# lucasjinreal/yolov7_d2

Hardware: AMD Instinct MI355X
Metric: images/sec training, YOLOX-s 640x640 bs=16/GPU (higher is better)
Workload: dtype bf16; 1 GPU; YOLOX-s CSPDarknet+PAFPN 640x640 bs=16/GPU: fwd + SimOTA loss + bwd + grad all-reduce + SGD(momentum) step, uint8 image batch + labels resident in HBM; global_batch=16, parallelism=dp1, hipgraph=True

## Files before the change

yolov7_d2_amd/csrc/conv1x1_stream.h:

```cpp
#pragma once
#include "common.h"
#include "conv_bn.h"

#define C1_MAX_SLICES 16
#define C1_MAX_BN 2
struct C1Slice {
  const u32x4* w;
  __bf16* y;
  double* stats;
  int wld, ldy, sld, nslots;
  int bnj, c0;
  const float* bias;
  const __bf16* aux;
  int ldaux, pad2_;
};
struct C1K {
  const __bf16* x;
  int ldx, ntiles, nco, nb;
  int xcd_order, dbg;
  C1Slice s[C1_MAX_SLICES];
  CBnFwd bn[C1_MAX_BN];
  const BnXf* xf;
  int xfw, pad_;
  int relu, epi;
  int npix, ragged;
};
struct C1Launch {
  int K, WM, PT, NBUF, MODE, grid, lds, XF;
  C1K k;
};

#define C1_VMCNT(n) asm volatile("s_waitcnt vmcnt(%0)" ::"n"(n) : "memory")

static __device__ uint4 g_c1_zero_page[4];
static __device__ __attribute__((aligned(256))) unsigned g_c1_bar[MI_BN_BAR_WORDS];

__device__ __forceinline__ void c1_glds16(const void* sbase, unsigned voff, unsigned lds_off) {
  asm volatile("s_mov_b32 m0, %2\n\ts_nop 4\n\tglobal_load_lds_dwordx4 %0, %1" ::"v"(voff), "s"(sbase),
               "s"(lds_off)
               : "memory");
}

template <int K, int WM, int WN, int PT, int NBUF, int MODE, int XF = 0>
__global__ __launch_bounds__(WM* WN * 64) void c1s_kernel(const C1K p) {
  static_assert(!XF || MODE == 1, "the input transform comes with the forward (statistics) mode");
  constexpr int NW = WM * WN, TPIX = WN * PT * 32, KC8 = K / 8, KS = K / 16, R = K * 2;
  constexpr int XB = TPIX * R;
  constexpr int D = XB / (1024 * NW);
  static_assert(D >= 1 && XB % (1024 * NW) == 0, "tile / DMA split");
  constexpr int RPI = KC8 >= 64 ? 1 : 64 / KC8;
  constexpr int RBSH = K >= 128 ? 0 : (K == 64 ? 1 : 2);
  constexpr int SWM = KC8 - 1 < 15 ? KC8 - 1 : 15;
  constexpr int S = 2 * PT;
  constexpr bool AUXM = MODE == 2 || MODE == 5 || MODE == 6;
  constexpr bool RAGGED_OK = (MODE == 0 || MODE == 2 || MODE >= 4) && !XF;
  constexpr bool BIASM = MODE == 4 || MODE == 5;
  constexpr int L = MODE == 6 ? 4 * PT : (AUXM ? 2 * PT : 0);
  constexpr int W0 = (NBUF - 2) * D + L;
  constexpr int W1 = NBUF > 2 ? (NBUF - 2) * D + (S + L) + L : (S + L);
  constexpr int W2 = NBUF > 3 ? (NBUF - 2) * D + 2 * (S + L) + L : (NBUF - 2) * D + (NBUF - 1) * (S + L);
  constexpr int W3 = (NBUF - 2) * D + (NBUF - 1) * (S + L);
  static_assert(W3 < 64 && W2 < 64, "vmcnt field");
  constexpr int X1 = NBUF > 2 ? (NBUF - 3) * D + (2 * D + S) : S;
  constexpr int X2 = NBUF > 3 ? (NBUF - 4) * D + 2 * (2 * D + S) : (NBUF - 1) * S + (NBUF - 2) * 2 * D;
  constexpr int X3 = (NBUF - 1) * S + (NBUF - 2) * 2 * D;
  static_assert(!XF || (X3 < 64 && X2 < 64 && X1 < 64), "vmcnt field");

  extern __shared__ __attribute__((aligned(16))) char smem[];
  const unsigned lds0 = (unsigned)(uintptr_t)(__attribute__((address_space(3))) char*)smem;
  const int tid = threadIdx.x, lane = tid & 63;
  const int wave = __builtin_amdgcn_readfirstlane(tid >> 6);
  const int wm = wave / WN, wn = wave % WN;
  const int l31 = lane & 31, h = lane >> 5;
  const int nb = p.nb;
  const int cot = p.xcd_order ? (int)blockIdx.x / nb : (int)blockIdx.x % p.nco;
  const int b = p.xcd_order ? (int)blockIdx.x % nb : (int)blockIdx.x / p.nco;
  const int nt = (p.ntiles - b + nb - 1) / nb;
  const C1Slice sl = p.s[cot * WM + wm];
  unsigned gen0 = 0;
  if constexpr (MODE == 3) {
    const int nblk = (int)gridDim.x;
    if (tid == 0)
      gen0 = __hip_atomic_load(bn_bar_gen(g_c1_bar, (int)blockIdx.x % (nblk < BN_BAR_G ? nblk : BN_BAR_G)), __ATOMIC_RELAXED, __HIP_MEMORY_SCOPE_AGENT);
  }
  constexpr bool STATS = MODE == 1 || MODE == 3;

  bf16x8 a[KS];
#pragma unroll
  for (int ks = 0; ks < KS; ++ks) a[ks] = __builtin_bit_cast(bf16x8, sl.w[(size_t)(ks * 2 + h) * sl.wld + l31]);

  const int ldxb = p.ldx * 2;
  unsigned doff[D];
#pragma unroll
  for (int d = 0; d < D; ++d) {
    const int q = wave * D + d;
    const int row = q * RPI + (KC8 >= 64 ? 0 : lane / KC8);
    const int c = KC8 >= 64 ? lane : lane % KC8;
    doff[d] = (unsigned)(row * ldxb + ((c ^ ((row >> RBSH) & SWM)) << 4));
  }
  const size_t xtile = (size_t)TPIX * (size_t)ldxb;
  auto issue_x = [&](int i, int buf) {
    const bool live = i < nt;
    const char* xt = live ? (const char*)p.x + (size_t)(b + i * nb) * xtile : (const char*)g_c1_zero_page;
    if (RAGGED_OK && live && p.ragged && b + i * nb == p.ntiles - 1) {
      const int lim = p.npix - (p.ntiles - 1) * TPIX;
#pragma unroll
      for (int d = 0; d < D; ++d) {
        const int q = wave * D + d;
        const int row = q * RPI + (KC8 >= 64 ? 0 : lane / KC8);
        const int c = KC8 >= 64 ? lane : lane % KC8;
        c1_glds16(xt, row < lim ? doff[d] : (unsigned)(c << 4), lds0 + buf * XB + (wave * D + d) * 1024);
      }
      return;
    }
#pragma unroll
    for (int d = 0; d < D; ++d) c1_glds16(xt, live ? doff[d] : 0u, lds0 + buf * XB + (wave * D + d) * 1024);
  };

  unsigned brow[PT], bsw[PT];
#pragma unroll
  for (int j = 0; j < PT; ++j) {
    const int r = (wn * PT + j) * 32 + l31;
    brow[j] = (unsigned)(r * R);
    bsw[j] = (unsigned)((h ^ ((r >> RBSH) & SWM)) << 4);
  }
  const int ldyb = sl.ldy * 2;
  unsigned yoff[PT];
#pragma unroll
  for (int j = 0; j < PT; ++j) yoff[j] = (unsigned)(((wn * PT + j) * 32 + l31) * ldyb + h * 16);
  const size_t ytile = (size_t)TPIX * (size_t)ldyb;
  const int ldab5 = (MODE == 5 || MODE == 6) ? sl.ldaux * 2 : 0;
  unsigned aoff5[PT];
#pragma unroll
  for (int j = 0; j < PT; ++j) aoff5[j] = (unsigned)(((wn * PT + j) * 32 + l31) * ldab5 + h * 16);
  const size_t atile5 = (size_t)TPIX * (size_t)ldab5;
  float bs[BIASM ? 16 : 1];
  if constexpr (BIASM) {
#pragma unroll
    for (int q = 0; q < 4; ++q)
#pragma unroll
      for (int e = 0; e < 4; ++e) bs[4 * q + e] = sl.bias ? sl.bias[8 * q + 4 * h + e] : 0.f;
  }
  const bool relu4 = BIASM && p.relu != 0;

  float s1[16], s2[16];
  if constexpr (STATS) {
#pragma unroll
    for (int r = 0; r < 16; ++r) s1[r] = s2[r] = 0.f;
  }

#pragma unroll
  for (int i = 0; i < NBUF - 1; ++i) issue_x(i, i);

  float* const s_sc = (float*)(smem + NBUF * XB);
  float* const s_sh = s_sc + K;
  int xf_act = 0, xf_ldab = 0;
  char* xf_a = nullptr;
  if constexpr (XF) {
    bnx_tables(p.xf, s_sc, s_sh, NW * 64, blockIdx.x == 0);
    xf_act = p.xf->bn.act;
    xf_ldab = p.xf->bn.lda * 2;
    xf_a = (p.xfw && cot == 0) ? (char*)p.xf->bn.a : nullptr;
    __syncthreads();
  }

  int buf = 0, nbuf = NBUF - 1;
  for (int i = 0; i < nt; ++i) {
    char* const yt = (char*)sl.y + (size_t)(b + i * nb) * ytile;
    int lim = TPIX;
    if constexpr (RAGGED_OK) {
      if (p.ragged && b + i * nb == p.ntiles - 1) lim = p.npix - (p.ntiles - 1) * TPIX;
    }
    u32x4 old[2 * PT];
    u32x4 aux6[MODE == 6 ? 2 * PT : 1];
    if constexpr (MODE == 2 || MODE == 6) {
#pragma unroll
      for (int j = 0; j < PT; ++j) {
        const unsigned yo = ((wn * PT + j) * 32 + l31) < lim ? yoff[j] : (unsigned)(h * 16);
        asm volatile("s_nop 4\n\tglobal_load_dwordx4 %0, %1, %2" : "=v"(old[j * 2]) : "v"(yo), "s"(yt) : "memory");
        asm volatile("global_load_dwordx4 %0, %1, %2 offset:32" : "=v"(old[j * 2 + 1]) : "v"(yo), "s"(yt) : "memory");
      }
    }
    if constexpr (MODE == 5) {
      const char* const at5 = (const char*)sl.aux + (size_t)(b + i * nb) * atile5;
#pragma unroll
      for (int j = 0; j < PT; ++j) {
        const unsigned ao = ((wn * PT + j) * 32 + l31) < lim ? aoff5[j] : (unsigned)(h * 16);
        asm volatile("s_nop 4\n\tglobal_load_dwordx4 %0, %1, %2" : "=v"(old[j * 2]) : "v"(ao), "s"(at5) : "memory");
        asm volatile("global_load_dwordx4 %0, %1, %2 offset:32" : "=v"(old[j * 2 + 1]) : "v"(ao), "s"(at5) : "memory");
      }
    }
    if constexpr (MODE == 6) {
      const char* const at5 = (const char*)sl.aux + (size_t)(b + i * nb) * atile5;
#pragma unroll
      for (int j = 0; j < PT; ++j) {
        const unsigned ao = ((wn * PT + j) * 32 + l31) < lim ? aoff5[j] : (unsigned)(h * 16);
        asm volatile("s_nop 4\n\tglobal_load_dwordx4 %0, %1, %2" : "=v"(aux6[j * 2]) : "v"(ao), "s"(at5) : "memory");
        asm volatile("global_load_dwordx4 %0, %1, %2 offset:32" : "=v"(aux6[j * 2 + 1]) : "v"(ao), "s"(at5) : "memory");
      }
    }
    if (XF && xf_a) {
      if (i == 0) C1_VMCNT(W0);
      else if (i == 1) C1_VMCNT(X1);
      else if (i == 2) C1_VMCNT(X2);
      else C1_VMCNT(X3);
    } else {
      if (i == 0) C1_VMCNT(W0);
      else if (i == 1) C1_VMCNT(W1);
      else if (i == 2) C1_VMCNT(W2);
      else C1_VMCNT(W3);
    }
    if constexpr (XF) {
      char* const Xw = smem + buf * XB;
      char* const at = xf_a + (size_t)(b + i * nb) * ((size_t)TPIX * (size_t)xf_ldab);
#pragma unroll 2
      for (int d = 0; d < D; ++d) {
        const int q = wave * D + d;
        const int row = q * RPI + (KC8 >= 64 ? 0 : lane / KC8);
        const int c = KC8 >= 64 ? lane : lane % KC8;
        const int cg = c ^ ((row >> RBSH) & SWM);
        const u32x4 o = bnx_apply_lds(Xw + q * 1024 + lane * 16, s_sc, s_sh, cg, xf_act, true);
        if (xf_a) *(u32x4*)(at + (unsigned)(row * xf_ldab + cg * 16)) = o;
      }
      asm volatile("s_waitcnt lgkmcnt(0)" ::: "memory");
    }
    __builtin_amdgcn_s_barrier();
    issue_x(i + NBUF - 1, nbuf);

    f32x16 acc[PT];
#pragma unroll
    for (int j = 0; j < PT; ++j)
#pragma unroll
      for (int r = 0; r < 16; ++r) acc[j][r] = 0.f;
    const char* Xs = smem + buf * XB;
#pragma unroll
    for (int ks = 0; ks < KS; ++ks) {
      bf16x8 bf[PT];
#pragma unroll
      for (int j = 0; j < PT; ++j) bf[j] = __builtin_bit_cast(bf16x8, *(const u32x4*)(Xs + brow[j] + ((unsigned)(ks * 32) ^ bsw[j])));
#pragma unroll
      for (int j = 0; j < PT; ++j) acc[j] = __builtin_amdgcn_mfma_f32_32x32x16_bf16(a[ks], bf[j], acc[j], 0, 0, 0);
    }

    if constexpr (AUXM) {
      if constexpr (MODE == 6) {
        if constexpr (PT == 1)
          asm volatile("s_waitcnt vmcnt(%4)" : "+v"(old[0]), "+v"(old[1]), "+v"(aux6[0]), "+v"(aux6[1]) : "n"(D) : "memory");
        else
          asm volatile("s_waitcnt vmcnt(%8)"
                       : "+v"(old[0]), "+v"(old[1]), "+v"(old[2]), "+v"(old[3]), "+v"(aux6[0]), "+v"(aux6[1]), "+v"(aux6[2]), "+v"(aux6[3])
                       : "n"(D) : "memory");
      } else if constexpr (PT == 1)
        asm volatile("s_waitcnt vmcnt(%2)" : "+v"(old[0]), "+v"(old[1]) : "n"(D) : "memory");
      else
        asm volatile("s_waitcnt vmcnt(%4)" : "+v"(old[0]), "+v"(old[1]), "+v"(old[2]), "+v"(old[3]) : "n"(D) : "memory");
    }
#pragma unroll
    for (int j = 0; j < PT; ++j) {
      unsigned pk[8];
#pragma unroll
      for (int q = 0; q < 4; ++q) {
        bf16x4 o;
#pragma unroll
        for (int e = 0; e < 4; ++e) {
          if constexpr (BIASM) {
            float v = acc[j][4 * q + e] + bs[4 * q + e];
            if (relu4) v = fmaxf(v, 0.f);
            o[e] = (__bf16)v;
          } else {
            o[e] = (__bf16)acc[j][4 * q + e];
          }
        }
        if constexpr (STATS) {
#pragma unroll
          for (int e = 0; e < 4; ++e) {
            const float f = (float)o[e];
            s1[4 * q + e] += f;
            s2[4 * q + e] = __builtin_fmaf(f, f, s2[4 * q + e]);
          }
        }
        const u32x2 u = __builtin_bit_cast(u32x2, o);
        pk[2 * q] = u[0];
        pk[2 * q + 1] = u[1];
      }
#pragma unroll
      for (int pr = 0; pr < 2; ++pr) {
        const int q0 = 2 * pr, q1 = 2 * pr + 1;
        const auto w0 = __builtin_amdgcn_permlane32_swap(pk[2 * q0], pk[2 * q1], false, false);
        const auto w1 = __builtin_amdgcn_permlane32_swap(pk[2 * q0 + 1], pk[2 * q1 + 1], false, false);
        u32x4 v = {w0[0], w1[0], w0[1], w1[1]};
        if constexpr (MODE == 5) {
          const bf16x8 nv = __builtin_bit_cast(bf16x8, v), ov = __builtin_bit_cast(bf16x8, old[j * 2 + pr]);
          bf16x8 rv;
          if (p.epi == 1) {
#pragma unroll
            for (int e = 0; e < 8; ++e) rv[e] = (__bf16)fmaxf((float)(__bf16)((float)nv[e] + (float)ov[e]), 0.f);
          } else {
#pragma unroll
            for (int e = 0; e < 8; ++e) rv[e] = (float)ov[e] > 0.f ? nv[e] : (__bf16)0.f;
          }
          v = __builtin_bit_cast(u32x4, rv);
        }
        if constexpr (MODE == 2 || MODE == 6) {
          const bf16x8 nv = __builtin_bit_cast(bf16x8, v), ov = __builtin_bit_cast(bf16x8, old[j * 2 + pr]);
          bf16x8 rv;
#pragma unroll
          for (int e = 0; e < 8; ++e) rv[e] = (__bf16)((float)nv[e] + (float)ov[e]);
          if constexpr (MODE == 6) {
            const bf16x8 mv = __builtin_bit_cast(bf16x8, aux6[j * 2 + pr]);
#pragma unroll
            for (int e = 0; e < 8; ++e) rv[e] = (float)mv[e] > 0.f ? rv[e] : (__bf16)0.f;
          }
          v = __builtin_bit_cast(u32x4, rv);
        }
        if (!RAGGED_OK || ((wn * PT + j) * 32 + l31) < lim) *(u32x4*)(yt + yoff[j] + pr * 32) = v;
      }
    }
    buf = buf + 1 == NBUF ? 0 : buf + 1;
    nbuf = nbuf + 1 == NBUF ? 0 : nbuf + 1;
  }

  C1_VMCNT(0);
  if constexpr (STATS) {
#pragma unroll
    for (int off = 1; off < 32; off <<= 1)
#pragma unroll
      for (int r = 0; r < 16; ++r) {
        s1[r] += __shfl_xor(s1[r], off, 64);
        s2[r] += __shfl_xor(s2[r], off, 64);
      }
    __syncthreads();
    float* red = (float*)smem;
    if (l31 == 0) {
#pragma unroll
      for (int r = 0; r < 16; ++r) {
        const int c = wm * 32 + 8 * (r >> 2) + 4 * h + (r & 3);
        red[(wn * WM * 32 + c) * 2 + 0] = s1[r];
        red[(wn * WM * 32 + c) * 2 + 1] = s2[r];
      }
    }
    __syncthreads();
    if (wave < WM && lane < 32) {
      float a1 = 0.f, a2 = 0.f;
#pragma unroll
      for (int q = 0; q < WN; ++q) {
        a1 += red[(q * WM * 32 + wave * 32 + lane) * 2 + 0];
        a2 += red[(q * WM * 32 + wave * 32 + lane) * 2 + 1];
      }
      const C1Slice so = p.s[cot * WM + wave];
      double* sp = so.stats + (size_t)((int)blockIdx.x % so.nslots) * so.sld + lane * 2;
      if (!(p.dbg & 1)) {
        atomicAdd(sp, (double)a1);
        atomicAdd(sp + 1, (double)a2);
      }
    }
  }
  if constexpr (MODE == 3) {
    int* const s_gave_up = (int*)(smem + 16384);
    bn_grid_barrier(g_c1_bar, gen0, (int)blockIdx.x, (int)gridDim.x, s_gave_up);
    const float poison = *s_gave_up ? __builtin_nanf("") : 0.f;
    const CBnFwd& bn = p.bn[sl.bnj];
    float scl, shl;
    cbn_finalize(bn, sl.stats + l31 * 2, sl.sld, sl.nslots, sl.c0 + l31, b == 0 && wn == 0 && h == 0, poison, scl, shl);
    float sc[2][8], sh[2][8];
#pragma unroll
    for (int pr = 0; pr < 2; ++pr)
#pragma unroll
      for (int e = 0; e < 8; ++e) {
        sc[pr][e] = __shfl(scl, pr * 16 + h * 8 + e, 64);
        sh[pr][e] = __shfl(shl, pr * 16 + h * 8 + e, 64);
      }
    const int act = bn.act;
    const bool has_res = bn.res != nullptr;
    const int ldab = bn.lda * 2, ldrb = bn.ldres * 2;
    unsigned aoff[PT], roff[PT];
#pragma unroll
    for (int j = 0; j < PT; ++j) {
      aoff[j] = (unsigned)(((wn * PT + j) * 32 + l31) * ldab + h * 16);
      roff[j] = (unsigned)(((wn * PT + j) * 32 + l31) * ldrb + h * 16);
    }
    char* const a0 = (char*)(bn.a + sl.c0);
    const char* const r0 = (const char*)(bn.res + sl.c0);
    const size_t atile = (size_t)TPIX * (size_t)ldab, rtile = (size_t)TPIX * (size_t)ldrb;
    for (int i = 0; i < nt; ++i) {
      const size_t t = (size_t)(b + i * nb);
      const char* const yt = (const char*)sl.y + t * ytile;
      char* const at = a0 + t * atile;
      const char* const rt = r0 + t * rtile;
      u32x4 v[2 * PT], r[2 * PT];
#pragma unroll
      for (int j = 0; j < PT; ++j)
#pragma unroll
        for (int pr = 0; pr < 2; ++pr) {
          v[j * 2 + pr] = *(const u32x4*)(yt + yoff[j] + pr * 32);
          r[j * 2 + pr] = has_res ? *(const u32x4*)(rt + roff[j] + pr * 32) : u32x4{0u, 0u, 0u, 0u};
        }
#pragma unroll
      for (int j = 0; j < PT; ++j)
#pragma unroll
        for (int pr = 0; pr < 2; ++pr)
          *(u32x4*)(at + aoff[j] + pr * 32) = cbn_apply8(v[j * 2 + pr], sc[pr], sh[pr], act, has_res, r[j * 2 + pr]);
    }
  }
}

template <int K, int WM, int WN, int PT, int NBUF, int MODE, int XF = 0>
static int c1s_launch_one(const C1Launch& l, hipStream_t s) {
  auto fn = c1s_kernel<K, WM, WN, PT, NBUF, MODE, XF>;
  static bool attr_done = false;
  if (!attr_done) {
    hipFuncSetAttribute((const void*)fn, hipFuncAttributeMaxDynamicSharedMemorySize, 160 * 1024);
    attr_done = true;
  }
  hipLaunchKernelGGL(fn, dim3((unsigned)l.grid), dim3(WM * WN * 64), (size_t)l.lds, s, l.k);
  MI_CHECK_LAUNCH("conv1x1_stream");
  return MI_OK;
}

constexpr int c1s_nbuf(int K, int tpix) { return tpix * K * 2 >= 65536 ? 2 : (tpix * K * 2 >= 32768 ? 3 : 4); }

constexpr bool c1s_valid(int K, int tpix) {
  return (tpix * K * 2) % 8192 == 0 && tpix * K * 2 * c1s_nbuf(K, tpix) <= 160 * 1024;
}

template <int K, int MODE, int XF = 0>
static int c1s_launch_k(const C1Launch& l, hipStream_t s) {
  if constexpr (c1s_valid(K, 128)) {
    if (l.WM == 4 && l.PT == 2) return c1s_launch_one<K, 4, 2, 2, c1s_nbuf(K, 128), MODE, XF>(l, s);
    if (l.WM == 2 && l.PT == 1) return c1s_launch_one<K, 2, 4, 1, c1s_nbuf(K, 128), MODE, XF>(l, s);
  }
  if constexpr (c1s_valid(K, 64)) {
    if (l.WM == 4 && l.PT == 1) return c1s_launch_one<K, 4, 2, 1, c1s_nbuf(K, 64), MODE, XF>(l, s);
  }
  if constexpr (c1s_valid(K, 256)) {
    if (l.WM == 1 && l.PT == 1) return c1s_launch_one<K, 1, 8, 1, c1s_nbuf(K, 256), MODE, XF>(l, s);
  }
  MI_FAIL(MI_EINVAL, "conv1x1_stream: no kernel for K %d WM %d PT %d", K, l.WM, l.PT);
}
```

yolov7_d2_amd/csrc/conv3x3_ws.h:

```cpp
#pragma once
#include "common.h"
#include "conv_bn.h"

#define W3_MAX_JOBS 8
#define W3_TW 16
template <int S, int TH>
struct W3Geo {
  static constexpr int HH = S == 1 ? TH + 2 : 2 * TH + 1;
  static constexpr int HW = S == 1 ? W3_TW + 2 : 2 * W3_TW + 1;
  static constexpr int HPIX = HH * HW;
  static constexpr int HROWS = (HPIX + 63) / 64 * 64;
  static constexpr int tap(int dy, int dx) { return S == 1 ? dy * HW + dx : dy * HW + (dx & 1) * (W3_TW + 1) + (dx >> 1); }
};

struct W3Job {
  const __bf16* x;
  const u32x4* w;
  __bf16* y;
  double* stats;
  int ldx, ldy, N, H, W, tilesY, tilesX, ntiles;
  int blk0, nblk;
  int wld, nslots, sld, pad_;
  int tw[9];
  int inH;
  CBnFwd bn;
  int inW, xfw;
  const BnXf* xf;
};
struct W3K {
  int njobs, dbg;
  W3Job j[W3_MAX_JOBS];
};
struct W3Launch {
  int K, MODE, grid, lds, S, XF;
  W3K k;
};

#define W3_VMCNT(n) asm volatile("s_waitcnt vmcnt(%0)" ::"n"(n) : "memory")

static __device__ uint4 g_w3_zero_page[4];
static __device__ __attribute__((aligned(256))) unsigned g_w3_bar[MI_BN_BAR_WORDS];

__device__ __forceinline__ void w3_glds16(const void* g, unsigned lds_off) {
  asm volatile("s_mov_b32 m0, %1\n\ts_nop 0\n\tglobal_load_lds_dwordx4 %0, off" ::"v"(g), "s"(lds_off) : "memory");
}

template <int K, int WM, int WN, int G, int MODE, int S = 1, int TH = 8, int XF = 0>
__global__ __launch_bounds__(WM* WN * 64, (K == 128 || (S == 2 && K == 64)) ? 1 : 2) void w3_kernel(const W3K p) {
  static_assert(!XF || MODE == 1, "the input transform comes with the forward (statistics) mode");
  constexpr int NW = WM * WN, KC8 = K / 8, KS = K / 16;
  using Geo = W3Geo<S, TH>;
  constexpr int W3_TH = TH, W3_HW = Geo::HW, W3_HPIX = Geo::HPIX, W3_HROWS = Geo::HROWS;
  static_assert(WN * G * 32 == W3_TH * W3_TW, "pixel tile");
  constexpr int PLANE = W3_HROWS * 16;
  constexpr int NQ = (W3_HROWS / 64) * KC8;
  constexpr int D = NQ / NW;
  static_assert(NQ % NW == 0 && D >= 1, "DMA split");
  constexpr int XB = KC8 * PLANE;
  static_assert((KC8 - 1) * PLANE + Geo::tap(2, 2) * 16 < 65536, "ds_read immediate");
  constexpr int NS = 9 * KS, NTS = NS / 3;
  constexpr int NST = 2 * G;
  constexpr int DST = 2 * (D - 1) < NTS ? 2 : 1, SST = 2 * NST + NST / 2 <= NTS ? 2 : 1;
  static_assert(DST * (D - 1) < NTS && SST * NST + (MODE == 2 ? NST / 2 : 0) <= NTS, "the memory operations of a tile fit its main loop");

  extern __shared__ __attribute__((aligned(16))) char smem[];
  const unsigned lds0 = (unsigned)(uintptr_t)(__attribute__((address_space(3))) char*)smem;
  const int tid = threadIdx.x, lane = tid & 63;
  const int wave = __builtin_amdgcn_readfirstlane(tid >> 6);
  const int wm = wave / WN, wn = wave % WN;
  const int l31 = lane & 31, h = lane >> 5;

  int ji = 0;
  while (ji + 1 < p.njobs && (int)blockIdx.x >= p.j[ji + 1].blk0) ++ji;
  ji = __builtin_amdgcn_readfirstlane(ji);
  const W3Job& jb = p.j[ji];
  const int b = (int)blockIdx.x - jb.blk0, nb = jb.nblk;
  const int nt = (jb.ntiles - b + nb - 1) / nb;
  constexpr bool STATS = MODE == 1 || MODE == 3;
  unsigned gen0 = 0;
  if constexpr (MODE == 3) {
    const int nblk = (int)gridDim.x;
    if (tid == 0)
      gen0 = __hip_atomic_load(bn_bar_gen(g_w3_bar, (int)blockIdx.x % (nblk < BN_BAR_G ? nblk : BN_BAR_G)), __ATOMIC_RELAXED, __HIP_MEMORY_SCOPE_AGENT);
  }
  const int H = jb.H, Wd = jb.W, tilesX = jb.tilesX, tpi = jb.tilesY * jb.tilesX;
  const int inH = S == 1 ? jb.H : jb.inH, inW = S == 1 ? jb.W : jb.inW;
  const int ldxb = jb.ldx * 2, ldyb = jb.ldy * 2;
  const char* const xbase = (const char*)jb.x;
  char* const ybase = (char*)jb.y;
  const char* zpage = (const char*)g_w3_zero_page;
  asm volatile("" : "+s"(zpage));
  float* const s_sc = (float*)(smem + 2 * (K / 8) * Geo::HROWS * 16 + 256 * 32 * 4);
  float* const s_sh = s_sc + K;
  int xf_act = 0, xf_ldab = 0;
  char* xf_a = nullptr;
  if constexpr (XF) {
    const BnXf* const xf = jb.xf;
    bnx_tables(xf, s_sc, s_sh, NW * 64, jb.xfw != 0 && b == 0);
    xf_act = xf->bn.act;
    xf_ldab = xf->bn.lda * 2;
    xf_a = jb.xfw ? (char*)xf->bn.a : nullptr;
  }

  bf16x8 a[9][KS];
  {
    const u32x4* wb = jb.w + wm * 32 + l31;
#pragma unroll
    for (int t = 0; t < 9; ++t) {
      const int slab = jb.tw[t] * KC8;
#pragma unroll
      for (int ks = 0; ks < KS; ++ks) a[t][ks] = __builtin_bit_cast(bf16x8, wb[(size_t)(slab + ks * 2 + h) * jb.wld]);
    }
  }

  struct Org { int img, ty0, tx0; };
  auto tile_origin = [&](int i) {
    const int t = b + i * nb;
    Org o;
    o.img = t / tpi;
    const int rem = t - o.img * tpi, tyq = rem / tilesX;
    o.ty0 = tyq * W3_TH;
    o.tx0 = (rem - tyq * tilesX) * W3_TW;
    return o;
  };
  auto issue_x1 = [&](const Org& o, int buf, int d) {
    const int iy0 = S * o.ty0 - 1, ix0 = S * o.tx0 - 1;
    const char* xt = xbase + ((size_t)o.img * inH * inW + (ptrdiff_t)iy0 * inW + ix0) * (ptrdiff_t)ldxb;
    const int q = wave * D + d;
    const int pb = q / KC8, k8 = q % KC8;
    const int pix = pb * 64 + lane;
    const int hy = S == 1 ? (int)(((unsigned)pix * 3641u) >> 16) : (int)(((unsigned)pix * 1986u) >> 16);
    const int hp = pix - hy * W3_HW;
    const int hx = S == 1 ? hp : (hp <= W3_TW ? 2 * hp : 2 * (hp - (W3_TW + 1)) + 1);
    const bool v = (pix < W3_HPIX) & ((unsigned)(iy0 + hy) < (unsigned)inH) & ((unsigned)(ix0 + hx) < (unsigned)inW);
    const char* g = v ? xt + (unsigned)((hy * inW + hx) * ldxb + k8 * 16) : zpage;
    w3_glds16(g, lds0 + buf * XB + k8 * PLANE + pb * 1024);
  };

  int lg, lidx;
  {
    const int l = l31;
    lg = ((l >= 4) & (l < 12)) | ((l >= 16) & (l < 20)) | (l >= 28);
    lidx = l - (l < 4 ? 0 : l < 12 ? 4 : l < 20 ? 8 : l < 28 ? 12 : 16);
  }
  unsigned bbase[G];
#pragma unroll
  for (int g = 0; g < G; ++g) bbase[g] = (unsigned)(h * PLANE + (S * ((wn * G + g) * 2 + lg) * W3_HW + lidx) * 16);
  auto out_ptr = [&](const Org& o, int g) -> char* {
    const int py = o.ty0 + (wn * G + g) * 2 + lg, px = o.tx0 + lidx;
    char* q = ybase + (((size_t)o.img * H + py) * Wd + px) * (size_t)ldyb + wm * 64 + h * 16;
    return ((py < H) & (px < Wd)) ? q : nullptr;
  };

  float* const sacc = (float*)(smem + 2 * XB) + tid * 4;
  constexpr int SAS = NW * 64 * 4;
  if constexpr (STATS) {
#pragma unroll
    for (int q = 0; q < 8; ++q) *(f32x4*)(sacc + q * SAS) = f32x4{0.f, 0.f, 0.f, 0.f};
  }

  Org oc = tile_origin(0), op = oc;
#pragma unroll
  for (int d = 0; d < D; ++d) issue_x1(oc, 0, d);

  u32x4 pk[NST];
#pragma unroll
  for (int q = 0; q < NST; ++q) pk[q] = u32x4{0u, 0u, 0u, 0u};
  for (int i = 0; i < nt; ++i) {
    W3_VMCNT(0);
    if constexpr (XF) {
      if (i == 0) __syncthreads();
      const int iy0 = S * oc.ty0 - 1, ix0 = S * oc.tx0 - 1;
      char* const Xw = smem + (i & 1) * XB;
      char* const at = xf_a + ((size_t)oc.img * inH * inW + (ptrdiff_t)iy0 * inW + ix0) * (ptrdiff_t)xf_ldab;
#pragma unroll 2
      for (int d = 0; d < D; ++d) {
        const int q = wave * D + d;
        const int pb = q / KC8, k8 = q % KC8;
        const int pix = pb * 64 + lane;
        const int hy = S == 1 ? (int)(((unsigned)pix * 3641u) >> 16) : (int)(((unsigned)pix * 1986u) >> 16);
        const int hp = pix - hy * W3_HW;
        const int hx = S == 1 ? hp : (hp <= W3_TW ? 2 * hp : 2 * (hp - (W3_TW + 1)) + 1);
        const bool v = (pix < W3_HPIX) & ((unsigned)(iy0 + hy) < (unsigned)inH) & ((unsigned)(ix0 + hx) < (unsigned)inW);
        const u32x4 o = bnx_apply_lds(Xw + k8 * PLANE + pb * 1024 + lane * 16, s_sc, s_sh, k8, xf_act, v);
        const bool inner = v & (hy >= 1) & (hy <= S * W3_TH) & (hx >= 1) & (hx <= S * W3_TW);
        if (xf_a && inner) *(u32x4*)(at + (unsigned)((hy * inW + hx) * xf_ldab + k8 * 16)) = o;
      }
      asm volatile("s_waitcnt lgkmcnt(0)" ::: "memory");
    }
    __builtin_amdgcn_s_barrier();
    const bool more = (i + 1 < nt) & !(p.dbg & 2);
    const bool prev = i > 0;
    const Org on = tile_origin(i + 1 < nt ? i + 1 : i);
    const char* Xs = smem + (i & 1) * XB;
    u32x4 old[NST];

    f32x16 acc[G];
#pragma unroll
    for (int g = 0; g < G; ++g)
#pragma unroll
      for (int r = 0; r < 16; ++r) acc[g][r] = 0.f;
    auto ldb = [&](int step, bf16x8(&dst)[G]) {
      const int t9 = step / KS, ks = step % KS, dy = t9 / 3, dx = t9 % 3;
#pragma unroll
      for (int g = 0; g < G; ++g)
        dst[g] = __builtin_bit_cast(bf16x8, *(const u32x4*)(Xs + bbase[g] + (2 * ks * PLANE + Geo::tap(dy, dx) * 16)));
    };
    bf16x8 bf[3][G];
    ldb(0, bf[0]);
    ldb(1, bf[1]);
    if (!(p.dbg & 4))
#pragma unroll
    for (int ts = 0; ts < NTS; ++ts) {
      if (ts % DST == 0 && ts / DST < D) {
        if (more) issue_x1(on, (i + 1) & 1, ts / DST);
      }
      if (ts % SST == SST - 1 && ts / SST < NST) {
        char* q = prev ? out_ptr(op, (ts / SST) / 2) : nullptr;
        if (q) *(u32x4*)(q + ((ts / SST) % 2) * 32) = pk[ts / SST];
      }
      if constexpr (MODE == 2) {
        if (ts >= SST * NST && ts < SST * NST + NST / 2) {
#pragma unroll
          for (int l = 2 * (ts - SST * NST); l < 2 * (ts - SST * NST) + 2; ++l) {
            char* q = out_ptr(oc, l / 2);
            old[l] = u32x4{0u, 0u, 0u, 0u};
            if (q) {
              if (l % 2 == 0) asm volatile("global_load_dwordx4 %0, %1, off" : "+v"(old[l]) : "v"(q) : "memory");
              else asm volatile("global_load_dwordx4 %0, %1, off offset:32" : "+v"(old[l]) : "v"(q) : "memory");
            }
          }
        }
      }
#pragma unroll
      for (int r = 0; r < 3; ++r) {
        const int st = 3 * ts + r;
        __builtin_amdgcn_sched_barrier(0);
        if (st + 2 < NS) ldb(st + 2, bf[(r + 2) % 3]);
#pragma unroll
        for (int g = 0; g < G; ++g)
          acc[g] = __builtin_amdgcn_mfma_f32_32x32x16_bf16(a[st / KS][st % KS], bf[r][g], acc[g], 0, 0, 0);
#pragma unroll
        for (int g = 0; g < G; ++g) {
          __builtin_amdgcn_sched_group_barrier(0x008, 1, 0);
          __builtin_amdgcn_sched_group_barrier(0x100, 1, 0);
          __builtin_amdgcn_sched_group_barrier(0x002, 2, 0);
        }
      }
      __builtin_amdgcn_sched_barrier(0);
    }

    if constexpr (MODE == 2) {
      if constexpr (NST == 2)
        asm volatile("s_waitcnt vmcnt(0)" : "+v"(old[0]), "+v"(old[1])::"memory");
      else if constexpr (NST == 4)
        asm volatile("s_waitcnt vmcnt(0)" : "+v"(old[0]), "+v"(old[1]), "+v"(old[2]), "+v"(old[3])::"memory");
      else
        asm volatile("s_waitcnt vmcnt(0)"
                     : "+v"(old[0]), "+v"(old[1]), "+v"(old[2]), "+v"(old[3]), "+v"(old[4]), "+v"(old[5]), "+v"(old[6]), "+v"(old[7])::"memory");
    }
    float s1[16], s2[16];
    if constexpr (STATS) {
#pragma unroll
      for (int q = 0; q < 4; ++q) {
        const f32x4 u = *(const f32x4*)(sacc + q * SAS), w = *(const f32x4*)(sacc + (4 + q) * SAS);
#pragma unroll
        for (int e = 0; e < 4; ++e) { s1[4 * q + e] = u[e]; s2[4 * q + e] = w[e]; }
      }
    }
#pragma unroll
    for (int g = 0; g < G; ++g) {
      bool pvg = true;
      if constexpr (STATS) pvg = out_ptr(oc, g) != nullptr;
      unsigned pw[8];
#pragma unroll
      for (int q = 0; q < 4; ++q) {
        bf16x4 o;
#pragma unroll
        for (int e = 0; e < 4; ++e) o[e] = (__bf16)acc[g][4 * q + e];
        if constexpr (STATS) {
#pragma unroll
          for (int e = 0; e < 4; ++e) {
            const float f = pvg ? (float)o[e] : 0.f;
            s1[4 * q + e] += f;
            s2[4 * q + e] = __builtin_fmaf(f, f, s2[4 * q + e]);
          }
        }
        const u32x2 u = __builtin_bit_cast(u32x2, o);
        pw[2 * q] = u[0];
        pw[2 * q + 1] = u[1];
      }
#pragma unroll
      for (int pr = 0; pr < 2; ++pr) {
        const int q0 = 2 * pr, q1 = 2 * pr + 1;
        const auto w0 = __builtin_amdgcn_permlane32_swap(pw[2 * q0], pw[2 * q1], false, false);
        const auto w1 = __builtin_amdgcn_permlane32_swap(pw[2 * q0 + 1], pw[2 * q1 + 1], false, false);
        u32x4 v = {w0[0], w1[0], w0[1], w1[1]};
        if constexpr (MODE == 2) {
          const bf16x8 nv = __builtin_bit_cast(bf16x8, v), ov = __builtin_bit_cast(bf16x8, old[g * 2 + pr]);
          bf16x8 rv;
#pragma unroll
          for (int e = 0; e < 8; ++e) rv[e] = (__bf16)((float)nv[e] + (float)ov[e]);
          v = __builtin_bit_cast(u32x4, rv);
        }
        pk[g * 2 + pr] = v;
      }
    }
    if constexpr (STATS) {
#pragma unroll
      for (int q = 0; q < 4; ++q) {
        *(f32x4*)(sacc + q * SAS) = f32x4{s1[4 * q], s1[4 * q + 1], s1[4 * q + 2], s1[4 * q + 3]};
        *(f32x4*)(sacc + (4 + q) * SAS) = f32x4{s2[4 * q], s2[4 * q + 1], s2[4 * q + 2], s2[4 * q + 3]};
      }
    }
    op = oc;
    oc = on;
  }
#pragma unroll
  for (int q = 0; q < NST; ++q) {
    char* o = out_ptr(op, q / 2);
    if (o) *(u32x4*)(o + (q % 2) * 32) = pk[q];
  }

  W3_VMCNT(0);
  if constexpr (STATS) {
    float s1[16], s2[16];
#pragma unroll
    for (int q = 0; q < 4; ++q) {
      const f32x4 u = *(const f32x4*)(sacc + q * SAS), w = *(const f32x4*)(sacc + (4 + q) * SAS);
#pragma unroll
      for (int e = 0; e < 4; ++e) { s1[4 * q + e] = u[e]; s2[4 * q + e] = w[e]; }
    }
#pragma unroll
    for (int off = 1; off < 32; off <<= 1)
#pragma unroll
      for (int r = 0; r < 16; ++r) {
        s1[r] += __shfl_xor(s1[r], off, 64);
        s2[r] += __shfl_xor(s2[r], off, 64);
      }
    __syncthreads();
    float* red = (float*)smem;
    if (l31 == 0) {
#pragma unroll
      for (int r = 0; r < 16; ++r) {
        const int c = wm * 32 + 8 * (r >> 2) + 4 * h + (r & 3);
        red[(wn * WM * 32 + c) * 2 + 0] = s1[r];
        red[(wn * WM * 32 + c) * 2 + 1] = s2[r];
      }
    }
    __syncthreads();
    if (tid < WM * 32) {
      float a1 = 0.f, a2 = 0.f;
#pragma unroll
      for (int q = 0; q < WN; ++q) {
        a1 += red[(q * WM * 32 + tid) * 2 + 0];
        a2 += red[(q * WM * 32 + tid) * 2 + 1];
      }
      double* sp = jb.stats + (size_t)((int)blockIdx.x % jb.nslots) * jb.sld + tid * 2;
      if (!(p.dbg & 1)) {
        atomicAdd(sp, (double)a1);
        atomicAdd(sp + 1, (double)a2);
      }
    }
  }
  if constexpr (MODE == 3) {
    int* const s_gave_up = (int*)(smem + 16384);
    bn_grid_barrier(g_w3_bar, gen0, (int)blockIdx.x, (int)gridDim.x, s_gave_up);
    const float poison = *s_gave_up ? __builtin_nanf("") : 0.f;
    const CBnFwd& bn = jb.bn;
    float scl, shl;
    cbn_finalize(bn, jb.stats + (wm * 32 + l31) * 2, jb.sld, jb.nslots, wm * 32 + l31, b == 0 && wn == 0 && h == 0, poison, scl, shl);
    float sc[2][8], sh[2][8];
#pragma unroll
    for (int pr = 0; pr < 2; ++pr)
#pragma unroll
      for (int e = 0; e < 8; ++e) {
        sc[pr][e] = __shfl(scl, pr * 16 + h * 8 + e, 64);
        sh[pr][e] = __shfl(shl, pr * 16 + h * 8 + e, 64);
      }
    const int act = bn.act;
    const bool has_res = bn.res != nullptr;
    const size_t ldab = (size_t)bn.lda * 2, ldrb = (size_t)bn.ldres * 2;
    char* const abase = (char*)bn.a + wm * 64 + h * 16;
    const char* const rbase = (const char*)bn.res + wm * 64 + h * 16;
    for (int i = 0; i < nt; ++i) {
      const Org o = tile_origin(i);
      u32x4 v[NST], r[NST];
      size_t pixi[G];
      bool ok[G];
#pragma unroll
      for (int g = 0; g < G; ++g) {
        const int py = o.ty0 + (wn * G + g) * 2 + lg, px = o.tx0 + lidx;
        ok[g] = (py < H) & (px < Wd);
        pixi[g] = ((size_t)o.img * H + py) * Wd + px;
#pragma unroll
        for (int pr = 0; pr < 2; ++pr) {
          v[g * 2 + pr] = r[g * 2 + pr] = u32x4{0u, 0u, 0u, 0u};
          if (ok[g]) {
            v[g * 2 + pr] = *(const u32x4*)(ybase + pixi[g] * (size_t)ldyb + wm * 64 + h * 16 + pr * 32);
            if (has_res) r[g * 2 + pr] = *(const u32x4*)(rbase + pixi[g] * ldrb + pr * 32);
          }
        }
      }
#pragma unroll
      for (int g = 0; g < G; ++g)
#pragma unroll
        for (int pr = 0; pr < 2; ++pr)
          if (ok[g]) *(u32x4*)(abase + pixi[g] * ldab + pr * 32) = cbn_apply8(v[g * 2 + pr], sc[pr], sh[pr], act, has_res, r[g * 2 + pr]);
    }
  }
}

template <int K, int WM, int WN, int G, int MODE, int S = 1, int TH = 8, int XF = 0>
static int w3_launch_one(const W3Launch& l, hipStream_t s) {
  auto fn = w3_kernel<K, WM, WN, G, MODE, S, TH, XF>;
  static bool attr_done = false;
  if (!attr_done) {
    hipFuncSetAttribute((const void*)fn, hipFuncAttributeMaxDynamicSharedMemorySize, 160 * 1024);
    attr_done = true;
  }
  hipLaunchKernelGGL(fn, dim3((unsigned)l.grid), dim3(WM * WN * 64), (size_t)l.lds, s, l.k);
  MI_CHECK_LAUNCH("conv3x3_ws");
  return MI_OK;
}
constexpr int w3_tile_h(int S, int K) { return S == 1 ? 8 : (K == 128 ? 2 : 4); }
constexpr int w3_block_cout(int S, int K) { return S == 1 ? K : (K == 32 ? 64 : 128); }
template <int MODE, int XF = 0>
static int w3_launch_mode(const W3Launch& l, hipStream_t s) {
  if (l.S == 2) {
    if constexpr (MODE == 1 || MODE == 0) {
      switch (l.K) {
        case 128: return w3_launch_one<128, 4, 1, 1, MODE, 2, 2, XF>(l, s);
        case 64: return w3_launch_one<64, 4, 1, 2, MODE, 2, 4, XF>(l, s);
        case 32: return w3_launch_one<32, 2, 2, 1, MODE, 2, 4, XF>(l, s);
      }
    }
    MI_FAIL(MI_EINVAL, "conv3x3_ws: stride 2 with K %d / mode %d", l.K, MODE);
  }
  switch (l.K) {
    case 128: return w3_launch_one<128, 4, 1, 4, MODE, 1, 8, XF>(l, s);
    case 64: return w3_launch_one<64, 2, 2, 2, MODE, 1, 8, XF>(l, s);
    case 32: return w3_launch_one<32, 1, 4, 1, MODE, 1, 8, XF>(l, s);
  }
  MI_FAIL(MI_EINVAL, "conv3x3_ws: K %d", l.K);
}
```

yolov7_d2_amd/csrc/conv_bn.h:

```cpp
#pragma once
#include "common.h"
#include "bn_common.h"

#define BN_FUS_SPIN_LIMIT (1 << 22)
#define BN_BAR_G MI_BN_BAR_GROUPS
__device__ __forceinline__ unsigned* bn_bar_gen(unsigned* bar, int g) { return bar + 64 * (1 + g); }
__device__ __forceinline__ unsigned* bn_bar_cnt(unsigned* bar, int g) { return bar + 64 * (1 + BN_BAR_G + g); }
__device__ __forceinline__ int bn_bar_group(const int bid, const int nb) { return bid % (nb < BN_BAR_G ? nb : BN_BAR_G); }
__device__ __forceinline__ bool bn_bar_count(unsigned* bar, const int bid, const int nb) {
  const int G = nb < BN_BAR_G ? nb : BN_BAR_G;
  const int g = bid % G;
  const unsigned gsize = (unsigned)((nb - g + G - 1) / G);
  if (__hip_atomic_fetch_add(bn_bar_cnt(bar, g), 1u, __ATOMIC_RELAXED, __HIP_MEMORY_SCOPE_AGENT) == gsize - 1u) {
    __hip_atomic_store(bn_bar_cnt(bar, g), 0u, __ATOMIC_RELAXED, __HIP_MEMORY_SCOPE_AGENT);
    if (__hip_atomic_fetch_add(bar, 1u, __ATOMIC_RELAXED, __HIP_MEMORY_SCOPE_AGENT) == (unsigned)G - 1u) {
      __hip_atomic_store(bar, 0u, __ATOMIC_RELAXED, __HIP_MEMORY_SCOPE_AGENT);
      return true;
    }
  }
  return false;
}
__device__ __forceinline__ void bn_bar_release(unsigned* bar, const int nb) {
  const int G = nb < BN_BAR_G ? nb : BN_BAR_G;
  for (int q = 0; q < G; ++q) __hip_atomic_fetch_add(bn_bar_gen(bar, q), 1u, __ATOMIC_RELAXED, __HIP_MEMORY_SCOPE_AGENT);
}
__device__ __forceinline__ bool bn_bar_wait(unsigned* bar, const unsigned gen0, const int bid, const int nb) {
  int spins = 0;
  while (__hip_atomic_load(bn_bar_gen(bar, bn_bar_group(bid, nb)), __ATOMIC_RELAXED, __HIP_MEMORY_SCOPE_AGENT) == gen0) {
    __builtin_amdgcn_s_sleep(8);
    if (++spins > BN_FUS_SPIN_LIMIT) {
      __hip_atomic_store(bar + 2, 1u, __ATOMIC_RELAXED, __HIP_MEMORY_SCOPE_AGENT);
      return true;
    }
  }
  return false;
}

__device__ __forceinline__ void bn_grid_barrier(unsigned* bar, const unsigned gen0, const int bid, const int nb, int* gave_up) {
  asm volatile("s_waitcnt vmcnt(0)" ::: "memory");
  __syncthreads();
  if (threadIdx.x == 0) {
    *gave_up = 0;
    if (bn_bar_count(bar, bid, nb)) bn_bar_release(bar, nb);
    else if (bn_bar_wait(bar, gen0, bid, nb)) *gave_up = 1;
  }
  __syncthreads();
}

__device__ __forceinline__ void bn_bar_arrive(unsigned* bar, const int bid, const int nb, int* gave_up, int* is_last) {
  asm volatile("s_waitcnt vmcnt(0)" ::: "memory");
  __syncthreads();
  if (threadIdx.x == 0) {
    *gave_up = 0;
    *is_last = bn_bar_count(bar, bid, nb) ? 1 : 0;
  }
  __syncthreads();
}
__device__ __forceinline__ void bn_bar_finish(unsigned* bar, const unsigned gen0, const int bid, const int nb, int* gave_up,
                                              const int* is_last) {
  asm volatile("s_waitcnt vmcnt(0)" ::: "memory");
  __syncthreads();
  if (threadIdx.x == 0) {
    if (*is_last) bn_bar_release(bar, nb);
    else if (bn_bar_wait(bar, gen0, bid, nb)) *gave_up = 1;
  }
  __syncthreads();
}


struct CBnFwd {
  const __bf16* res;
  __bf16* a;
  const float* gamma;
  const float* beta;
  float* rmean;
  float* rvar;
  long long* nbt;
  float* scale;
  float* shift;
  float* mean;
  float* invstd;
  int ldres, lda, act, pad_;
  double inv_count, unbias;
  float eps, momentum;
};

__device__ __forceinline__ void cbn_finalize(const CBnFwd& bn, const double* acc, int sld, int nslots, int c, bool writer,
                                             float poison, float& sc_out, float& sh_out) {
  double v1[MI_BN_SLOTS], v2[MI_BN_SLOTS];
#pragma unroll
  for (int k = 0; k < MI_BN_SLOTS; ++k) {
    if (k < nslots) {
      v1[k] = __hip_atomic_load(acc + (size_t)k * sld, __ATOMIC_RELAXED, __HIP_MEMORY_SCOPE_AGENT);
      v2[k] = __hip_atomic_load(acc + (size_t)k * sld + 1, __ATOMIC_RELAXED, __HIP_MEMORY_SCOPE_AGENT);
    } else {
      v1[k] = v2[k] = 0.0;
    }
  }
  double s1 = 0.0, s2 = 0.0;
#pragma unroll
  for (int k = 0; k < MI_BN_SLOTS; ++k) {
    s1 += v1[k];
    s2 += v2[k];
  }
  float sc, sh;
  const BnMoments m = bn_moments(s1, s2, bn.inv_count, bn.eps, bn.gamma[c], bn.beta[c], sc, sh);
  sc += poison;
  sh += poison;
  sc_out = sc;
  sh_out = sh;
  if (writer) bn_record<true>(bn, c, sc, sh, m, poison);
}

__device__ __forceinline__ u32x4 cbn_apply8(const u32x4 yv, const float* sc, const float* sh, const int act, const bool has_res,
                                            const u32x4 rv) {
  const bf16x8 v = __builtin_bit_cast(bf16x8, yv), r = __builtin_bit_cast(bf16x8, rv);
  float o[8];
#pragma unroll
  for (int e = 0; e < 8; ++e) {
    const float z = (float)v[e] * sc[e] + sh[e];
    o[e] = act ? z * sigmoidf_(z) : z;
  }
  if (has_res) {
#pragma unroll
    for (int e = 0; e < 8; ++e) o[e] += (float)r[e];
  }
  return __builtin_bit_cast(u32x4, pack8(o));
}

struct BnXf {
  CBnFwd bn;
  const double* acc;
  int sld, nslots, C, pad_;
};
static_assert(sizeof(BnXf) == sizeof(mi_bnx) && __builtin_offsetof(BnXf, acc) == __builtin_offsetof(mi_bnx, acc) &&
              __builtin_offsetof(BnXf, bn.inv_count) == __builtin_offsetof(mi_bnx, inv_count) &&
              __builtin_offsetof(BnXf, bn.lda) == __builtin_offsetof(mi_bnx, lda), "mi_bnx (include/mi355_det.h) mirrors BnXf");
__device__ __forceinline__ void bnx_tables(const BnXf* __restrict__ xf, float* s_sc, float* s_sh, const int nthreads, const bool rec) {
  const int C = xf->C, nslots = xf->nslots;
  const size_t sld2 = (size_t)(xf->sld >> 1);
  const CBnFwd& bn = xf->bn;
  for (int c = threadIdx.x; c < C; c += nthreads) {
    const f64x2* const ap = (const f64x2*)xf->acc + c;
    f64x2 v[MI_BN_SLOTS];
#pragma unroll
    for (int k = 0; k < MI_BN_SLOTS; ++k) v[k] = ap[(k < nslots ? (size_t)k : 0) * sld2];
    double s1 = 0.0, s2 = 0.0;
#pragma unroll
    for (int k = 0; k < MI_BN_SLOTS; ++k) {
      s1 += k < nslots ? v[k][0] : 0.0;
      s2 += k < nslots ? v[k][1] : 0.0;
    }
    float sc, sh;
    const BnMoments m = bn_moments(s1, s2, bn.inv_count, bn.eps, bn.gamma[c], bn.beta[c], sc, sh);
    s_sc[c] = sc;
    s_sh[c] = sh;
    if (rec) bn_record<true>(bn, c, sc, sh, m, BN_NO_POISON);
  }
}
__device__ __forceinline__ u32x4 bnx_apply_lds(char* sp, const float* s_sc, const float* s_sh, const int cg, const int act, const bool valid) {
  const u32x4 raw = *(const u32x4*)sp;
  const f32x4 c0 = *(const f32x4*)(s_sc + cg * 8), c1 = *(const f32x4*)(s_sc + cg * 8 + 4);
  const f32x4 h0 = *(const f32x4*)(s_sh + cg * 8), h1 = *(const f32x4*)(s_sh + cg * 8 + 4);
  const float sc[8] = {c0[0], c0[1], c0[2], c0[3], c1[0], c1[1], c1[2], c1[3]};
  const float sh[8] = {h0[0], h0[1], h0[2], h0[3], h1[0], h1[1], h1[2], h1[3]};
  u32x4 o = cbn_apply8(raw, sc, sh, act, false, u32x4{0u, 0u, 0u, 0u});
  if (!valid) o = u32x4{0u, 0u, 0u, 0u};
  *(u32x4*)sp = o;
  return o;
}
```

Measured before the change: 2945 images/sec.

## Streamline conv BN-stat block reduction with DPP transpose-fold and register stats

Replaces the per-register 5-step shfl_xor butterfly for BN statistics with a transpose-fold reduction that uses DPP lane swaps. Each lane ends up holding one channel's sum, which cuts cross-lane operations from 16x5 to about 8+4+2+1+1 per statistic. The block reduction is factored into a shared helper that skips LDS and barriers when WN==1. The 1x1 kernel no longer drains every outstanding store before the stats tail. For some 3x3 configurations, stats accumulate in registers instead of round-tripping through LDS, which adds register pressure in exchange.

```diff
diff --git a/yolov7_d2_amd/csrc/conv1x1_stream.h b/yolov7_d2_amd/csrc/conv1x1_stream.h
--- a/yolov7_d2_amd/csrc/conv1x1_stream.h
+++ b/yolov7_d2_amd/csrc/conv1x1_stream.h
@@ -65,6 +65,8 @@
   constexpr int X2 = NBUF > 3 ? (NBUF - 4) * D + 2 * (2 * D + S) : (NBUF - 1) * S + (NBUF - 2) * 2 * D;
   constexpr int X3 = (NBUF - 1) * S + (NBUF - 2) * 2 * D;
   static_assert(!XF || (X3 < 64 && X2 < 64 && X1 < 64), "vmcnt field");
+  constexpr int WT = S;
+  static_assert(WT < 64, "vmcnt field");
 
   extern __shared__ __attribute__((aligned(16))) char smem[];
   const unsigned lds0 = (unsigned)(uintptr_t)(__attribute__((address_space(3))) char*)smem;
@@ -320,40 +322,14 @@
     nbuf = nbuf + 1 == NBUF ? 0 : nbuf + 1;
   }
 
-  C1_VMCNT(0);
   if constexpr (STATS) {
-#pragma unroll
-    for (int off = 1; off < 32; off <<= 1)
-#pragma unroll
-      for (int r = 0; r < 16; ++r) {
-        s1[r] += __shfl_xor(s1[r], off, 64);
-        s2[r] += __shfl_xor(s2[r], off, 64);
-      }
-    __syncthreads();
-    float* red = (float*)smem;
-    if (l31 == 0) {
-#pragma unroll
-      for (int r = 0; r < 16; ++r) {
-        const int c = wm * 32 + 8 * (r >> 2) + 4 * h + (r & 3);
-        red[(wn * WM * 32 + c) * 2 + 0] = s1[r];
-        red[(wn * WM * 32 + c) * 2 + 1] = s2[r];
-      }
-    }
-    __syncthreads();
-    if (wave < WM && lane < 32) {
-      float a1 = 0.f, a2 = 0.f;
-#pragma unroll
-      for (int q = 0; q < WN; ++q) {
-        a1 += red[(q * WM * 32 + wave * 32 + lane) * 2 + 0];
-        a2 += red[(q * WM * 32 + wave * 32 + lane) * 2 + 1];
-      }
-      const C1Slice so = p.s[cot * WM + wave];
-      double* sp = so.stats + (size_t)((int)blockIdx.x % so.nslots) * so.sld + lane * 2;
-      if (!(p.dbg & 1)) {
-        atomicAdd(sp, (double)a1);
-        atomicAdd(sp + 1, (double)a2);
-      }
-    }
+    C1_VMCNT(WT);
+    cbn_block_stats<WM, WN>(s1, s2, (float*)smem, wave, lane, (p.dbg & 1) != 0, [&](const int c) {
+      const C1Slice& so = p.s[cot * WM + (c >> 5)];
+      return so.stats + (size_t)((int)blockIdx.x % so.nslots) * so.sld + (c & 31) * 2;
+    });
+  } else {
+    C1_VMCNT(0);
   }
   if constexpr (MODE == 3) {
     int* const s_gave_up = (int*)(smem + 16384);
diff --git a/yolov7_d2_amd/csrc/conv3x3_ws.h b/yolov7_d2_amd/csrc/conv3x3_ws.h
--- a/yolov7_d2_amd/csrc/conv3x3_ws.h
+++ b/yolov7_d2_amd/csrc/conv3x3_ws.h
@@ -152,11 +152,18 @@
     return ((py < H) & (px < Wd)) ? q : nullptr;
   };
 
+  constexpr bool SREG = (K == 32 && S == 1) || (K == 64 && S == 2);
   float* const sacc = (float*)(smem + 2 * XB) + tid * 4;
   constexpr int SAS = NW * 64 * 4;
+  float s1[16], s2[16];
   if constexpr (STATS) {
-#pragma unroll
-    for (int q = 0; q < 8; ++q) *(f32x4*)(sacc + q * SAS) = f32x4{0.f, 0.f, 0.f, 0.f};
+    if constexpr (SREG) {
+#pragma unroll
+      for (int r = 0; r < 16; ++r) s1[r] = s2[r] = 0.f;
+    } else {
+#pragma unroll
+      for (int q = 0; q < 8; ++q) *(f32x4*)(sacc + q * SAS) = f32x4{0.f, 0.f, 0.f, 0.f};
+    }
   }
 
   Org oc = tile_origin(0), op = oc;
@@ -259,8 +266,7 @@
         asm volatile("s_waitcnt vmcnt(0)"
                      : "+v"(old[0]), "+v"(old[1]), "+v"(old[2]), "+v"(old[3]), "+v"(old[4]), "+v"(old[5]), "+v"(old[6]), "+v"(old[7])::"memory");
     }
-    float s1[16], s2[16];
-    if constexpr (STATS) {
+    if constexpr (STATS && !SREG) {
 #pragma unroll
       for (int q = 0; q < 4; ++q) {
         const f32x4 u = *(const f32x4*)(sacc + q * SAS), w = *(const f32x4*)(sacc + (4 + q) * SAS);
@@ -306,7 +312,7 @@
         pk[g * 2 + pr] = v;
       }
     }
-    if constexpr (STATS) {
+    if constexpr (STATS && !SREG) {
 #pragma unroll
       for (int q = 0; q < 4; ++q) {
         *(f32x4*)(sacc + q * SAS) = f32x4{s1[4 * q], s1[4 * q + 1], s1[4 * q + 2], s1[4 * q + 3]};
@@ -322,46 +328,18 @@
     if (o) *(u32x4*)(o + (q % 2) * 32) = pk[q];
   }
 
-  W3_VMCNT(0);
   if constexpr (STATS) {
-    float s1[16], s2[16];
-#pragma unroll
-    for (int q = 0; q < 4; ++q) {
-      const f32x4 u = *(const f32x4*)(sacc + q * SAS), w = *(const f32x4*)(sacc + (4 + q) * SAS);
-#pragma unroll
-      for (int e = 0; e < 4; ++e) { s1[4 * q + e] = u[e]; s2[4 * q + e] = w[e]; }
-    }
-#pragma unroll
-    for (int off = 1; off < 32; off <<= 1)
-#pragma unroll
-      for (int r = 0; r < 16; ++r) {
-        s1[r] += __shfl_xor(s1[r], off, 64);
-        s2[r] += __shfl_xor(s2[r], off, 64);
-      }
-    __syncthreads();
-    float* red = (float*)smem;
-    if (l31 == 0) {
-#pragma unroll
-      for (int r = 0; r < 16; ++r) {
-        const int c = wm * 32 + 8 * (r >> 2) + 4 * h + (r & 3);
-        red[(wn * WM * 32 + c) * 2 + 0] = s1[r];
-        red[(wn * WM * 32 + c) * 2 + 1] = s2[r];
-      }
-    }
-    __syncthreads();
-    if (tid < WM * 32) {
-      float a1 = 0.f, a2 = 0.f;
-#pragma unroll
-      for (int q = 0; q < WN; ++q) {
-        a1 += red[(q * WM * 32 + tid) * 2 + 0];
-        a2 += red[(q * WM * 32 + tid) * 2 + 1];
-      }
-      double* sp = jb.stats + (size_t)((int)blockIdx.x % jb.nslots) * jb.sld + tid * 2;
-      if (!(p.dbg & 1)) {
-        atomicAdd(sp, (double)a1);
-        atomicAdd(sp + 1, (double)a2);
-      }
-    }
+    if constexpr (!SREG) {
+#pragma unroll
+      for (int q = 0; q < 4; ++q) {
+        const f32x4 u = *(const f32x4*)(sacc + q * SAS), w = *(const f32x4*)(sacc + (4 + q) * SAS);
+#pragma unroll
+        for (int e = 0; e < 4; ++e) { s1[4 * q + e] = u[e]; s2[4 * q + e] = w[e]; }
+      }
+    }
+    cbn_block_stats<WM, WN>(s1, s2, (float*)smem, wave, lane, (p.dbg & 1) != 0, [&](const int c) {
+      return jb.stats + (size_t)((int)blockIdx.x % jb.nslots) * jb.sld + c * 2;
+    });
   }
   if constexpr (MODE == 3) {
     int* const s_gave_up = (int*)(smem + 16384);
diff --git a/yolov7_d2_amd/csrc/conv_bn.h b/yolov7_d2_amd/csrc/conv_bn.h
--- a/yolov7_d2_amd/csrc/conv_bn.h
+++ b/yolov7_d2_amd/csrc/conv_bn.h
@@ -128,6 +128,69 @@
   return __builtin_bit_cast(u32x4, pack8(o));
 }
 
+template <int OFF>
+__device__ __forceinline__ float cbn_lane_xor(const float v) {
+  const int i = __builtin_bit_cast(int, v);
+  if constexpr (OFF == 1) return __builtin_bit_cast(float, __builtin_amdgcn_update_dpp(0, i, 0xB1, 0xF, 0xF, true));
+  else if constexpr (OFF == 2) return __builtin_bit_cast(float, __builtin_amdgcn_update_dpp(0, i, 0x4E, 0xF, 0xF, true));
+  else if constexpr (OFF == 8) return __builtin_bit_cast(float, __builtin_amdgcn_update_dpp(0, i, 0x128, 0xF, 0xF, true));
+  else return __shfl_xor(v, OFF, 64);
+}
+template <int N, int OFF>
+__device__ __forceinline__ void cbn_halve(const float (&in)[2 * N], float (&out)[N], const bool up) {
+#pragma unroll
+  for (int k = 0; k < N; ++k) {
+    const float keep = up ? in[k + N] : in[k], send = up ? in[k] : in[k + N];
+    out[k] = keep + cbn_lane_xor<OFF>(send);
+  }
+}
+__device__ __forceinline__ float cbn_fold32(const float (&s)[16], const int l31) {
+  float t8[8], t4[4], t2[2], t1[1];
+  cbn_halve<8, 1>(s, t8, (l31 & 1) != 0);
+  cbn_halve<4, 2>(t8, t4, (l31 & 2) != 0);
+  cbn_halve<2, 4>(t4, t2, (l31 & 4) != 0);
+  cbn_halve<1, 8>(t2, t1, (l31 & 8) != 0);
+  return t1[0] + cbn_lane_xor<16>(t1[0]);
+}
+template <int WM, int WN, class StatsOf>
+__device__ __forceinline__ void cbn_block_stats(const float (&s1)[16], const float (&s2)[16], float* red, const int wave,
+                                                const int lane, const bool noatom, StatsOf&& stats_of) {
+#ifdef MI_CONV_STATS_NOTAIL
+#pragma unroll
+  for (int r = 0; r < 16; ++r) asm volatile("" ::"v"(s1[r]), "v"(s2[r]));
+  return;
+#endif
+  const int wm = wave / WN, wn = wave % WN, l31 = lane & 31, h = lane >> 5;
+  const float f1 = cbn_fold32(s1, l31), f2 = cbn_fold32(s2, l31);
+  const int r = ((l31 & 1) << 3) | ((l31 & 2) << 1) | ((l31 & 4) >> 1) | ((l31 & 8) >> 3);
+  const int c = wm * 32 + 8 * (r >> 2) + 4 * h + (r & 3);
+  if constexpr (WN == 1) {
+    if (l31 < 16 && !noatom) {
+      double* sp = stats_of(c);
+      atomicAdd(sp, (double)f1);
+      atomicAdd(sp + 1, (double)f2);
+    }
+  } else {
+    double* const sp = stats_of((wave < WM ? wave : 0) * 32 + l31);
+    __syncthreads();
+    if (l31 < 16) *(float2*)(red + (wn * WM * 32 + c) * 2) = float2{f1, f2};
+    __syncthreads();
+    if (wave < WM && lane < 32) {
+      float a1 = 0.f, a2 = 0.f;
+#pragma unroll
+      for (int q = 0; q < WN; ++q) {
+        const float2 v = *(const float2*)(red + (q * WM * 32 + wave * 32 + lane) * 2);
+        a1 += v.x;
+        a2 += v.y;
+      }
+      if (!noatom) {
+        atomicAdd(sp, (double)a1);
+        atomicAdd(sp + 1, (double)a2);
+      }
+    }
+  }
+}
+
 struct BnXf {
   CBnFwd bn;
   const double* acc;
```

Measured after the change: 3023 images/sec, median of 6. 1.03x the previous value.
